# OpenSLAM-org/openslam_g2o

Measured on AMD Instinct MI355X. Metric: linear-solve ms/iter (buildSystem + setLambda + solve + restoreDiagonal), 100k-pose BA, lower is better.
Workload: dtype f64; 1 GPU; synthetic BA (BASELINE.json configs[3]): 100000 poses / 1000000 landmarks / 5000000 observations, BlockSolver_6_3 semantics, Schur + multifrontal block Cholesky, lambda=10; poses=100000, landmarks=1000000, edges=5000000, parallelism=1 GPU, edge_data=estimates+measurements in HBM, errors/Jacobians evaluated inside buildSystem, information=identity, declared for the whole edge set (not read per edge)

## Files before the change

openslam_g2o_amd/csrc/block_solver.h:

```cpp
#pragma once
#include <cstring>
#include <memory>

#include "common.h"
#include "comm.h"
#include "block_pcg.h"
#include "sparse_cholesky.h"

namespace g2ohip {

struct EdgeSet {
  int d = 0, n = 0, dim0 = 0, dim1 = 0;
  bool unary = false;
  int parts = 0;
  std::vector<int> v0, v1;
  int kernel_kind = 0;
  double delta = 1.0;
  DevBuf<double> rk;
  const double *J0 = nullptr, *J1 = nullptr, *omega = nullptr, *err = nullptr;
  DevBuf<double> own_J0, own_J1, own_omega, own_err;
  bool has_data = false;
  bool external = false;
  bool has_err = false;
  DevBuf<int> vp_ptr, vp_ent, vl_ptr, vl_ent;
// ... 283 lines not shown
  void pg_bind_landmark_edges(const char* who, int set, int type, const int* pose_vertex, const int* point_vertex, const double* meas,
                              const double* info, const double* offset, const double* kcam);
  struct EstimateTable {
    DevBuf<double> val, bak;
    DevBuf<int> hidx;
    std::vector<int> h_hidx;
    int n = 0, stride = 0;
    size_t scalars() const { return (size_t)n * stride; }
    bool same(int count, int str, const int* h) const {
      return count == n && str == stride && val.p && std::memcmp(h_hidx.data(), h, sizeof(int) * (size_t)n) == 0;
    }
    void set_values(const double* v, hipStream_t st) { val.upload(v, scalars(), st); }
    void commit(int count, int str, const double* v, const int* h, hipStream_t st) {
      n = count;
      stride = str;
      h_hidx.assign(h, h + count);
      val.upload(v, scalars(), st);
      hidx.upload(h, (size_t)count, st);
      bak.alloc(scalars());
    }
    void push(hipStream_t st) { copy(bak.p, val.p, st); }
    void pop(hipStream_t st) { copy(val.p, bak.p, st); }
    void download(double* h, hipStream_t st) const { val.download(h, scalars(), st); }
    void copy(double* dst, const double* src, hipStream_t st) const {
      if (n > 0) G2OHIP_HIP_CHECK(hipMemcpyAsync(dst, src, scalars() * sizeof(double), hipMemcpyDeviceToDevice, st));
    }
  };
  struct BaFrontEnd {
    int set = -1, n_edges = 0;
    EstimateTable cams, pts;
    double f = 0, cx = 0, cy = 0;
    bool stereo = false;
    double baseline = 0;
    int n_classes = 1;
    DevBuf<double> ctab;
    std::vector<double> h_ctab;
    DevBuf<int> cam_v, pt_v, edge_hpl;
    std::vector<int> h_cam_v, h_pt_v;
    long est_version = 0, bak_version = 0, sys_version = -1;
    int sys_kind = 0;
    double sys_delta = 0.0;
    bool omega_identity = false;
    bool err_valid = false, jac_valid = false;
    DevBuf<double> chi_part;
    bool fused_ok = false;
    DevBuf<double> meas;
    DevBuf<double> meas_pm, omega_pm;
    DevBuf<int> pt_pm, cam_pm;
    DevBuf<double> meas_lm, omega_lm;
    DevBuf<int> cam_q, pt_q;
    DevBuf<double> meas_q, omega_q;
    DevBuf<int> cam_lm, pt_lm, hpl_lm, row_lm;
    DevBuf<int4> ll_rec;
    DevBuf<int> ll_edge;
    DevBuf<int> ll_row;
    DevBuf<double> ll_meas, ll_omega;
    DevBuf<int4> tile_ll;
    DevBuf<int> sel_idx;
    DevBuf<double> sel_out;
    bool ll_slots_ok = false;
    bool has_backup = false;
  } ba_;
  struct PgFrontEnd {
    int set = -1, type = 0;
    DevBuf<int> vi, vj;
    std::vector<int> h_vi, h_vj;
    DevBuf<double> meas;
    EstimateTable poses;
    bool has_backup = false;
    bool err_valid = false, jac_valid = false;
    int lm_set = -1, lm_type = 0;
    DevBuf<int> vp, vl;
    std::vector<int> h_vp, h_vl;
    DevBuf<double> lm_meas;
    EstimateTable points;
    double offset[12] = {1, 0, 0, 0, 1, 0, 0, 0, 1, 0, 0, 0};
    double kcam[4] = {1, 1, 0, 0};
    int pr_set = -1, pr_type = 0;
    DevBuf<int> vq;
    std::vector<int> h_vq;
    DevBuf<double> pr_meas;
    double pr_offset[12] = {1, 0, 0, 0, 1, 0, 0, 0, 1, 0, 0, 0};
  } pg_;
  EventTimer tq_, ts_, tn_, tl_, tb_, tfe_;
  void require_structure() const;
  double reduce_sum_finish(int nblocks);
};

}
```

openslam_g2o_amd/csrc/block_solver.hip:

```cpp
#include "block_solver.h"

#include <algorithm>
#include <atomic>
#include <chrono>
#include <cmath>
#include <cstring>
#include <numeric>

namespace g2ohip {

namespace {

constexpr int kThreads = 256;
constexpr int kMaxBlocks = 1024;

template <int CTRL>
__device__ __forceinline__ double dpp_permute(double v) {
  const int lo = __double2loint(v), hi = __double2hiint(v);
  const int lo2 = __builtin_amdgcn_update_dpp(lo, lo, CTRL, 0xf, 0xf, true);
  const int hi2 = __builtin_amdgcn_update_dpp(hi, hi, CTRL, 0xf, 0xf, true);
  return __hiloint2double(hi2, lo2);
}
template <int G>
__device__ __forceinline__ double group_sum(double v) {
// ... 957 lines not shown
#pragma unroll
  for (int c = 0; c < 3; ++c)
#pragma unroll
    for (int r = 0; r < 3; ++r) {
      double t = 0.0;
#pragma unroll
      for (int m = 0; m < 3; ++m) t += Om[r + 3 * m] * Om[m + 3 * c];
      Om2[r + 3 * c] = t;
    }
  double a, b, cc;
  const bool small = theta < 0.00001;
  if (!small) {
    a = sin(theta) / theta;
    b = (1.0 - cos(theta)) / (theta * theta);
    cc = (theta - sin(theta)) / (theta * theta * theta);
  } else {
    a = 1.0; b = 1.0; cc = 1.0;
  }
#pragma unroll
  for (int i = 0; i < 9; ++i) {
    const double I = (i % 4 == 0) ? 1.0 : 0.0;
    R[i] = I + a * Om[i] + b * Om2[i];
    V[i] = small ? R[i] : I + b * Om[i] + cc * Om2[i];
  }
  double Rn[9], tn[3];
#pragma unroll
  for (int c = 0; c < 3; ++c)
#pragma unroll
    for (int r = 0; r < 3; ++r) {
      double t = 0.0;
#pragma unroll
      for (int m = 0; m < 3; ++m) t += R[r + 3 * m] * T[m + 3 * c];
      Rn[r + 3 * c] = t;
    }
#pragma unroll
  for (int r = 0; r < 3; ++r)
    tn[r] = R[r] * T[9] + R[r + 3] * T[10] + R[r + 6] * T[11] + V[r] * u[3] + V[r + 3] * u[4] + V[r + 6] * u[5];
#pragma unroll
  for (int i = 0; i < 9; ++i) T[i] = Rn[i];
  T[9] = tn[0]; T[10] = tn[1]; T[11] = tn[2];
}
__global__ void __launch_bounds__(kThreads) ba_update_pts_kernel(int np, double* __restrict__ pts, const int* __restrict__ hidx,
                                                               const double* __restrict__ xl) {
  const int t = blockIdx.x * blockDim.x + threadIdx.x;
  if (t >= np * 3) return;
  const int v = t / 3, c = t % 3;
  const int h = hidx[v];
  if (h >= 0) pts[t] += xl[(size_t)h * 3 + c];
}

struct BaEdgeLin {
  double A[6], B[12], r[2], O[4], w;
};
__device__ __forceinline__ void ba_edge_linearize(const double* __restrict__ T, const double* __restrict__ X, const double* __restrict__ z2,
                                                  const double* __restrict__ Op, double f, double cx, double cy, int kind, double delta,
                                                  bool want_A, BaEdgeLin& L) {
  const double x = T[0] * X[0] + T[3] * X[1] + T[6] * X[2] + T[9];
  const double y = T[1] * X[0] + T[4] * X[1] + T[7] * X[2] + T[10];
  const double z = T[2] * X[0] + T[5] * X[1] + T[8] * X[2] + T[11];
  const double iz = 1.0 / z;
  L.r[0] = z2[0] - (x * iz * f + cx);
  L.r[1] = z2[1] - (y * iz * f + cy);
  L.O[0] = Op[0]; L.O[1] = Op[1]; L.O[2] = Op[2]; L.O[3] = Op[3];
  const double Or0 = L.O[0] * L.r[0] + L.O[2] * L.r[1], Or1 = L.O[1] * L.r[0] + L.O[3] * L.r[1];
  L.w = robust_weight(kind, delta, L.r[0] * Or0 + L.r[1] * Or1);
  const double fz = f * iz, xz = x * iz, yz = y * iz;
  if (want_A) {
    const double tmp[6] = {f, 0.0, -xz * f, 0.0, f, -yz * f};
#pragma unroll
    for (int rr = 0; rr < 2; ++rr)
#pragma unroll
      for (int c = 0; c < 3; ++c) {
        double t = 0.0;
#pragma unroll
        for (int m = 0; m < 3; ++m) t += tmp[rr * 3 + m] * T[m + 3 * c];
        L.A[rr + 2 * c] = -iz * t;
      }
  }
  L.B[0 + 2 * 0] = xz * yz * f;          L.B[0 + 2 * 1] = -(1.0 + xz * xz) * f; L.B[0 + 2 * 2] = yz * f;
  L.B[0 + 2 * 3] = -fz;                  L.B[0 + 2 * 4] = 0.0;                  L.B[0 + 2 * 5] = xz * fz;
  L.B[1 + 2 * 0] = (1.0 + yz * yz) * f;  L.B[1 + 2 * 1] = -xz * yz * f;         L.B[1 + 2 * 2] = -xz * f;
  L.B[1 + 2 * 3] = 0.0;                  L.B[1 + 2 * 4] = -fz;                  L.B[1 + 2 * 5] = yz * fz;
}

__device__ __forceinline__ void ba_lm_accumulate(const BaEdgeLin& L, double (&H)[9], double (&b)[3], double (&OA)[6]) {
  const double w = L.w;
  const double O00 = w * L.O[0], O10 = w * L.O[1], O01 = w * L.O[2], O11 = w * L.O[3];
#pragma unroll
  for (int c = 0; c < 3; ++c) {
    OA[0 + 2 * c] = O00 * L.A[0 + 2 * c] + O01 * L.A[1 + 2 * c];
    OA[1 + 2 * c] = O10 * L.A[0 + 2 * c] + O11 * L.A[1 + 2 * c];
  }
  const double Or0 = O00 * L.r[0] + O01 * L.r[1], Or1 = O10 * L.r[0] + O11 * L.r[1];
#pragma unroll
  for (int c = 0; c < 3; ++c) {
    b[c] -= L.A[0 + 2 * c] * Or0 + L.A[1 + 2 * c] * Or1;
#pragma unroll
    for (int a = 0; a < 3; ++a) H[a + 3 * c] += L.A[0 + 2 * a] * OA[0 + 2 * c] + L.A[1 + 2 * a] * OA[1 + 2 * c];
  }
}
__device__ __forceinline__ void ba_hpl_block(const BaEdgeLin& L, const double (&OA)[6], double (&blk)[18]) {
#pragma unroll
  for (int c = 0; c < 3; ++c)
#pragma unroll
    for (int a = 0; a < 6; ++a) blk[a + 6 * c] = L.B[0 + 2 * a] * OA[0 + 2 * c] + L.B[1 + 2 * a] * OA[1 + 2 * c];
}

#ifndef G2OHIP_ASMLM_OCC
#define G2OHIP_ASMLM_OCC 4
#endif
template <int G, bool CLS = false>
__global__ void __launch_bounds__(kThreads, G2OHIP_ASMLM_OCC) ba_assemble_landmarks_kernel(
    int nL, const int* __restrict__ vptr, const int* __restrict__ vent, const double* __restrict__ cams, const double* __restrict__ pts,
    const int* __restrict__ cam_lm, const int* __restrict__ pt_lm, const double* __restrict__ meas_lm, const double* __restrict__ omega_lm,
    const int* __restrict__ hpl_lm, double f, double cx, double cy, int kind, double delta, double* __restrict__ Hll,
    double* __restrict__ bl, double* __restrict__ Hpl, double* __restrict__ err, int ident, const int* __restrict__ pl_colptr,
    int write_hpl, const double* __restrict__ ctab) {
  __shared__ __attribute__((aligned(16))) double stage[kThreads / 64][64 * 18];
// ... 294 lines not shown
    const int* __restrict__ row_lm, double f, double cx, double cy, int kind, double delta, int ident,
    const double* __restrict__ Dinv, const double* __restrict__ bl, const double* __restrict__ xp, double* __restrict__ xl,
    const double* __restrict__ ctab) {
  const int gt = blockIdx.x * blockDim.x + threadIdx.x;
  const int lm = gt / G, g = gt % G;
  const bool active = lm < nL;
  double c[3] = {0.0, 0.0, 0.0};
  const int k0 = active ? vptr[lm] : 0, k1 = active ? vptr[lm + 1] : 0;
  for (int k = k0 + g; k < k1; k += G) {
    const int row = row_lm[k];
    if (row < 0) continue;
    double T[12], X[3], z2[2], Op[4], xv[6];
    const double* Xp = pts + (size_t)pt_lm[k] * 3;
    X[0] = Xp[0]; X[1] = Xp[1]; X[2] = Xp[2];
    load_vec<12>(cams + (size_t)ba_edge_class<CLS>(cam_lm[k], ctab, f, cx, cy, kind, delta) * 12, T);
    load_vec<2>(meas_lm + (size_t)k * 2, z2);
    load_vec<6>(xp + (size_t)row * 6, xv);
    if (ident) {
      Op[0] = Op[3] = 1.0;
      Op[1] = Op[2] = 0.0;
    } else {
      load_vec<4>(omega_lm + (size_t)k * 4, Op);
    }
    BaEdgeLin L;
    ba_edge_linearize(T, X, z2, Op, f, cx, cy, kind, delta, true, L);
    double t0 = 0.0, t1 = 0.0;
#pragma unroll
    for (int a = 0; a < 6; ++a) {
      t0 += L.B[0 + 2 * a] * xv[a];
      t1 += L.B[1 + 2 * a] * xv[a];
    }
    const double w = L.w;
    const double u0 = w * (L.O[0] * t0 + L.O[2] * t1), u1 = w * (L.O[1] * t0 + L.O[3] * t1);
#pragma unroll
    for (int j = 0; j < 3; ++j) c[j] -= L.A[0 + 2 * j] * u0 + L.A[1 + 2 * j] * u1;
  }
  if (G > 1) {
#pragma unroll
    for (int j = 0; j < 3; ++j) c[j] = group_sum<G>(c[j]);
  }
  if (!active || g >= 3) return;
  double cl[3];
#pragma unroll
  for (int j = 0; j < 3; ++j) cl[j] = c[j] + bl[(size_t)lm * 3 + j];
  const double* D = Dinv + (size_t)lm * 9;
  if (G == 1) {
#pragma unroll
    for (int i = 0; i < 3; ++i) xl[(size_t)lm * 3 + i] = D[i] * cl[0] + D[i + 3] * cl[1] + D[i + 6] * cl[2];
  } else {
    xl[(size_t)lm * 3 + g] = D[g] * cl[0] + D[g + 3] * cl[1] + D[g + 6] * cl[2];
  }
}

template <bool CLS>
__global__ void __launch_bounds__(kThreads) ba_back_substitute_slots_kernel(
    const int* __restrict__ tile_lm0, const int4* __restrict__ tile_ll, const int4* __restrict__ ll_rec, const int* __restrict__ ll_row,
    const double* __restrict__ ll_meas, const double* __restrict__ ll_omega, const double* __restrict__ cams,
    const double* __restrict__ pts, double f, double cx, double cy, int kind, double delta, int ident, const double* __restrict__ Dinv,
    const double* __restrict__ bl, const double* __restrict__ xp, double* __restrict__ xl, const double* __restrict__ ctab) {
  const int t = blockIdx.x, tid = threadIdx.x, NT = blockDim.x;
  const int l0 = tile_lm0[(size_t)t * 8];
  const int4 tl = tile_ll[t];
  for (int sb = 0; sb < tl.y; sb += NT) {
    const int si = sb + tid;
    const size_t sg = (size_t)tl.x + min(si, tl.y - 1);
    int4 rc = ll_rec[sg];
    if (si >= tl.y) rc.x = (int)0x80000fffu;
    const int ent = rc.x;
    const int krel = ent & 0xfff, K = (ent >> 12) & 0xff, lmi = (ent >> 20) & 0x7ff;
    const bool head = ent >= 0;
    const int pos = head ? 0 : lmi;
    const int row = krel != 0xfff ? ll_row[sg] : -1;
    double c[3] = {0.0, 0.0, 0.0};
    {
      double T[12], X[3], z2[2], Op[4], xv[6];
      const double* Xp = pts + (size_t)rc.z * 3;
      X[0] = Xp[0]; X[1] = Xp[1]; X[2] = Xp[2];
      load_vec<12>(cams + (size_t)ba_edge_class<CLS>(rc.y, ctab, f, cx, cy, kind, delta) * 12, T);
      load_vec<2>(ll_meas + sg * 2, z2);
      load_vec<6>(xp + (size_t)max(row, 0) * 6, xv);
      if (ident) {
        Op[0] = Op[3] = 1.0;
        Op[1] = Op[2] = 0.0;
      } else {
        load_vec<4>(ll_omega + sg * 4, Op);
      }
      if (row >= 0) {
        BaEdgeLin L;
        ba_edge_linearize(T, X, z2, Op, f, cx, cy, kind, delta, true, L);
        double t0 = 0.0, t1 = 0.0;
#pragma unroll
        for (int a = 0; a < 6; ++a) {
          t0 += L.B[0 + 2 * a] * xv[a];
          t1 += L.B[1 + 2 * a] * xv[a];
        }
        const double w = L.w;
        const double u0 = w * (L.O[0] * t0 + L.O[2] * t1), u1 = w * (L.O[1] * t0 + L.O[3] * t1);
#pragma unroll
        for (int j = 0; j < 3; ++j) c[j] = -(L.A[0 + 2 * j] * u0 + L.A[1 + 2 * j] * u1);
      }
    }
    for (int d = 1; d < tl.w; d <<= 1) {
      const bool take = pos + d < K;
#pragma unroll
      for (int i = 0; i < 3; ++i) {
        const double o = __shfl_down(c[i], d);
        if (take) c[i] += o;
      }
    }
    if (head) {
      const int lm = l0 + lmi;
      double cl[3];
#pragma unroll
      for (int j = 0; j < 3; ++j) cl[j] = c[j] + bl[(size_t)lm * 3 + j];
      const double* D = Dinv + (size_t)lm * 9;
#pragma unroll
      for (int i = 0; i < 3; ++i) xl[(size_t)lm * 3 + i] = D[i] * cl[0] + D[i + 3] * cl[1] + D[i + 6] * cl[2];
    }
  }
}

#ifndef G2OHIP_ASMP_OCC
#define G2OHIP_ASMP_OCC 2
#endif
template <int G, bool CLS = false>
__global__ void __launch_bounds__(kThreads, G2OHIP_ASMP_OCC) ba_assemble_poses_kernel(
    int nP, const int* __restrict__ vptr, const double* __restrict__ cams, const double* __restrict__ pts,
    const int* __restrict__ cam_pm, const int* __restrict__ pt_pm, const double* __restrict__ meas_pm, const double* __restrict__ omega_pm,
    double f, double cx, double cy, int kind, double delta, double* __restrict__ Hpp, const int* __restrict__ diag_blk,
    double* __restrict__ bp, int accumulate, int ident, const int* __restrict__ act, const double* __restrict__ ctab) {
  const int gt = blockIdx.x * blockDim.x + threadIdx.x;
  const int vi_ = gt / G, g = gt % G;
  const bool active = vi_ < nP;
  const int v = (act && active) ? act[vi_] : vi_;
  double H[21], b[6];
#pragma unroll
  for (int i = 0; i < 21; ++i) H[i] = 0.0;
#pragma unroll
  for (int i = 0; i < 6; ++i) b[i] = 0.0;
  const int k0 = active ? vptr[v] : 0, k1 = active ? vptr[v + 1] : 0;
  double T[12];
  const int kf = k0 + g;
  if (kf < k1) load_vec<12>(cams + (size_t)(cam_pm[kf] & (CLS ? 0xffffff : -1)) * 12, T);
  int pt1 = kf < k1 ? pt_pm[kf] : 0, pt2 = kf + G < k1 ? pt_pm[kf + G] : 0;
  double Xn[3] = {0.0, 0.0, 0.0}, z2n[2] = {0.0, 0.0}, Opn[4] = {1.0, 0.0, 0.0, 1.0};
  if (kf < k1) {
    const double* Xp = pts + (size_t)pt1 * 3;
    Xn[0] = Xp[0]; Xn[1] = Xp[1]; Xn[2] = Xp[2];
    load_vec<2>(meas_pm + (size_t)kf * 2, z2n);
    if (!ident) load_vec<4>(omega_pm + (size_t)kf * 4, Opn);
  }
  for (int k = kf; k < k1; k += G) {
    double X[3], z2[2], Op[4];
    X[0] = Xn[0]; X[1] = Xn[1]; X[2] = Xn[2];
    z2[0] = z2n[0]; z2[1] = z2n[1];
#pragma unroll
    for (int i = 0; i < 4; ++i) Op[i] = Opn[i];
    {
      const int kn = k + G, kn2 = k + 2 * G;
      const int pt3 = kn2 < k1 ? pt_pm[kn2] : 0;
      if (kn < k1) {
        const double* Xp = pts + (size_t)pt2 * 3;
        Xn[0] = Xp[0]; Xn[1] = Xp[1]; Xn[2] = Xp[2];
        load_vec<2>(meas_pm + (size_t)kn * 2, z2n);
        if (!ident) load_vec<4>(omega_pm + (size_t)kn * 4, Opn);
      }
      pt2 = pt3;
    }
    if constexpr (CLS) (void)ba_edge_class<true>(cam_pm[k], ctab, f, cx, cy, kind, delta);
    BaEdgeLin L;
    ba_edge_linearize(T, X, z2, Op, f, cx, cy, kind, delta, false, L);
// ... 2293 lines not shown
  return v;
}

double BlockSolver::max_diagonal_sharded() {
  require_structure();
  G2OHIP_HIP_CHECK(hipSetDevice(device_));
  ensure_ll();
  const size_t np = (size_t)nP_ * p_;
  DevBuf<double> diag;
  diag.alloc(np);
  hipLaunchKernelGGL(gather_diag_kernel, dim3(grid_for(np)), dim3(kThreads), 0, st_, nP_, p_, d_Hpp.p, d_pp_diag.p, 0.0, diag.p);
  comm.all_reduce(diag.p, np, 0, st_);
  double m = 0.0;
  {
    const int nblocks = std::min(1024, grid_for(np));
    hipLaunchKernelGGL(max_partial_kernel, dim3(nblocks), dim3(kThreads), 0, st_, np, diag.p, d_red.p);
    std::vector<double> h(nblocks);
    d_red.download(h.data(), nblocks, st_);
    for (double v : h) m = std::max(m, v + lam_pose_);
  }
  double ml = 0.0;
  if (nL_ > 0) {
    const int nblocks = std::min(1024, grid_for((size_t)nL_ * l_));
    hipLaunchKernelGGL(maxdiag_partial_kernel, dim3(nblocks), dim3(kThreads), 0, st_, nL_, l_, d_Hll.p, (const int*)nullptr, d_red.p);
    std::vector<double> h(nblocks);
    d_red.download(h.data(), nblocks, st_);
    for (double v : h) ml = std::max(ml, v + lam_lm_);
  }
  comm.all_reduce_host(&ml, 1, 1, st_);
  return std::max(m, ml);
}

void BlockSolver::partition_info(int* pose_owner, int* block_consumer) {
  require_structure();
  const CholSymbolic& S = chol_->symbolic();
  if (pose_owner) std::copy(S.pose_owner.begin(), S.pose_owner.end(), pose_owner);
  if (block_consumer) std::copy(S.block_consumer.begin(), S.block_consumer.end(), block_consumer);
}

void BlockSolver::solve_back_substitute() {
  require_structure();
  if (!schur_) return;
  G2OHIP_HIP_CHECK(hipSetDevice(device_));
  solve_back_substitute_impl();
}

void BlockSolver::solve_back_substitute_impl() {
  if (profiling) tb_.start(st_);
  const size_t sizeP = (size_t)nP_ * p_;
  prof.begin(KernelProf::kBackSub, st_);
  if (ba_recompute_ok()) {
    EdgeSet& es = *sets_[ba_.set];
    const int GL = ba_lm_group();
    if (ba_fuse_landmarks && ba_.ll_slots_ok && n_tiles_ > 0) {
      with_bool(ba_.n_classes > 1, [&](auto cls) {
        constexpr bool CLS = cls;
        hipLaunchKernelGGL((ba_back_substitute_slots_kernel<CLS>), dim3(n_tiles_), dim3(kThreads), 0, st_, d_tile_lm0.p, ba_.tile_ll.p,
                           ba_.ll_rec.p, ba_.ll_row.p, ba_.ll_meas.p, ba_.ll_omega.p, ba_.cams.val.p, ba_.pts.val.p, ba_.f, ba_.cx, ba_.cy,
                           es.kernel_kind, es.delta, ba_.omega_identity ? 1 : 0, d_Dinv.p, d_b.p + sizeP, d_x.p, d_x.p + sizeP, ba_.ctab.p);
      });
    } else {
      const auto launch = [&](auto g, auto cls) {
        constexpr int GG = g;
        constexpr bool CLS = cls;
        hipLaunchKernelGGL((ba_back_substitute_kernel<GG, CLS>), dim3(grid_for((size_t)nL_ * GG)), dim3(kThreads), 0, st_, nL_, es.vl_ptr.p,
                           ba_.cams.val.p, ba_.pts.val.p, ba_.cam_lm.p, ba_.pt_lm.p, ba_.meas_lm.p, ba_.omega_lm.p, ba_.row_lm.p, ba_.f,
                           ba_.cx, ba_.cy, es.kernel_kind, es.delta, ba_.omega_identity ? 1 : 0, d_Dinv.p, d_b.p + sizeP, d_x.p,
                           d_x.p + sizeP, ba_.ctab.p);
      };
      if (ba_.n_classes > 1) launch(ic<8>, std::true_type{});
      else with_lane_group<1, 4, 8>(GL, [&](auto g) { launch(g, std::false_type{}); });
    }
  } else {
    ensure_hpl();
    const auto row = [&](auto p, auto l) {
      constexpr int P = p, L = l;
      if (p_ != P || l_ != L) return false;
      hipLaunchKernelGGL((back_substitute_kernel<P, L>), dim3(grid_for(nL_)), dim3(kThreads), 0, st_, nL_, d_pl_colptr.p,
                         d_pl_row.p, d_Hpl.p, d_Dinv.p, d_b.p + sizeP, d_x.p, d_x.p + sizeP);
      return true;
    };
    if (!(row(ic<6>, ic<3>) || row(ic<3>, ic<2>) || row(ic<7>, ic<3>) || row(ic<6>, ic<2>) || row(ic<3>, ic<3>)))
      throw ArgFailure("unsupported (pose_dim, landmark_dim)");
  }
  prof.end(KernelProf::kBackSub, st_);
  G2OHIP_HIP_CHECK(hipGetLastError());
  if (profiling) {
    tb_.stop(st_);
    times.backsub = tb_.seconds();
  }
}

template <int PD, int LD>
__global__ void __launch_bounds__(kThreads) mf_pose_kernel(int nP, const int* __restrict__ pm_ptr, const int* __restrict__ pm_q,
                                                         const int* __restrict__ pm_lm, const double* __restrict__ Hpl,
                                                         const double* __restrict__ tl, const double* init,
                                                         const double* __restrict__ dvec, const double* __restrict__ lam, double sign,
                                                         double* out) {
  const int t = blockIdx.x * blockDim.x + threadIdx.x;
  if (t >= nP * PD) return;
  const int i = t / PD, r = t - i * PD;
  double acc = 0.0;
  for (int k = pm_ptr[i]; k < pm_ptr[i + 1]; ++k) {
    const double* B = Hpl + (size_t)pm_q[k] * PD * LD + r;
    const double* tv = tl + (size_t)pm_lm[k] * LD;
#pragma unroll
    for (int c = 0; c < LD; ++c) acc += B[PD * c] * tv[c];
  }
  double v = init[t];
  if (dvec) v += lam[0] * dvec[t];
  out[t] = v + sign * acc;
}
template <int PD, int LD>
// ... 352 lines not shown
      ensure_ll();
      d_Hll.download(h, (size_t)nL_ * l_ * l_, st_);
      if (lam_lm_ != 0.0)
        for (size_t j = 0; j < (size_t)nL_; ++j)
          for (int i = 0; i < l_; ++i) h[j * l_ * l_ + i * (l_ + 1)] += lam_lm_;
      break;
    case 3: ensure_hschur(); d_Hschur.download(h, hs_row.size() * p_ * p_, st_); break;
    case 4: d_Dinv.download(h, (size_t)nL_ * l_ * l_, st_); break;
    default: throw ArgFailure("bad matrix selector");
  }
}
void BlockSolver::ba_set_edges(int set, const int* cam_vertex, const int* point_vertex, const double* meas, const double* info,
                               double f, double cx, double cy) {
  ba_set_edges_classes(set, cam_vertex, point_vertex, meas, info, f, cx, cy, 1, nullptr, nullptr);
}

__global__ void ba_gather_blocks_kernel(size_t n, const int* __restrict__ edge_hpl, const int* __restrict__ cam_v, const int* __restrict__ pt_v,
                                        const double* __restrict__ meas, const double* __restrict__ omega, int* __restrict__ cam_q,
                                        int* __restrict__ pt_q, double* __restrict__ meas_q, double* __restrict__ omega_q) {
  const size_t k = (size_t)blockIdx.x * blockDim.x + threadIdx.x;
  if (k >= n) return;
  const int q = edge_hpl[k];
  if (q < 0) return;
  cam_q[q] = cam_v[k];
  pt_q[q] = pt_v[k];
  meas_q[2 * (size_t)q] = meas[2 * k];
  meas_q[2 * (size_t)q + 1] = meas[2 * k + 1];
  if (omega_q)
    for (int i = 0; i < 4; ++i) omega_q[4 * (size_t)q + i] = omega[4 * k + i];
}
__global__ void ba_gather_lists_kernel(size_t n, const int* __restrict__ ent, const int* __restrict__ cam_v, const int* __restrict__ pt_v,
                                       const double* __restrict__ meas, const double* __restrict__ omega, const int* __restrict__ edge_hpl,
                                       const int* __restrict__ v1, int* __restrict__ cam_o, int* __restrict__ pt_o,
                                       double* __restrict__ meas_o, double* __restrict__ omega_o, int* __restrict__ hpl_o,
                                       int* __restrict__ row_o) {
  const size_t k = (size_t)blockIdx.x * blockDim.x + threadIdx.x;
  if (k >= n) return;
  const size_t e = (size_t)(ent[k] >> 1);
  cam_o[k] = cam_v[e];
  pt_o[k] = pt_v[e];
  meas_o[2 * k] = meas[2 * e];
  meas_o[2 * k + 1] = meas[2 * e + 1];
  if (omega_o)
    for (int i = 0; i < 4; ++i) omega_o[4 * k + i] = omega[4 * e + i];
  if (hpl_o) {
    const int h = edge_hpl[e];
    hpl_o[k] = h;
    row_o[k] = h >= 0 ? v1[e] : -1;
  }
}
__global__ void ba_gather_slots_kernel(const int4* __restrict__ tile_ll, const int* __restrict__ slots, const int* __restrict__ vl_ent,
                                       const int* __restrict__ cam_lm, const int* __restrict__ pt_lm, const int* __restrict__ hpl_lm,
                                       const int* __restrict__ row_lm, const double* __restrict__ meas_lm, const double* __restrict__ omega_lm,
                                       int4* __restrict__ rec, int* __restrict__ edge, int* __restrict__ srow, double* __restrict__ ms,
                                       double* __restrict__ os) {
  const int4 tl = tile_ll[blockIdx.x];
  for (int i = threadIdx.x; i < tl.y; i += blockDim.x) {
    const size_t sidx = (size_t)tl.x + i;
    const int w = slots[sidx];
    int4 r = make_int4(w, 0, 0, -1);
    int ed = 0, row = -1;
    double m0 = 0.0, m1 = 0.0, o[4] = {0.0, 0.0, 0.0, 0.0};
    if ((w & 0xfff) != 0xfff) {
      const size_t k = (size_t)tl.z + (w & 0xfff);
      r = make_int4(w, cam_lm[k], pt_lm[k], hpl_lm[k]);
      ed = vl_ent[k] >> 1;
      row = row_lm[k];
      m0 = meas_lm[2 * k];
      m1 = meas_lm[2 * k + 1];
      if (os)
        for (int j = 0; j < 4; ++j) o[j] = omega_lm[4 * k + j];
    }
    rec[sidx] = r;
    edge[sidx] = ed;
    srow[sidx] = row;
    ms[2 * sidx] = m0;
    ms[2 * sidx + 1] = m1;
    if (os)
      for (int j = 0; j < 4; ++j) os[4 * sidx + j] = o[j];
  }
}

void BlockSolver::ba_set_edges_classes(int set, const int* cam_vertex, const int* point_vertex, const double* meas, const double* info,
                                       double f, double cx, double cy, int n_classes, const double* class_params, const int* edge_class) {
  invalidate_graphs();
  require_structure();
  if (set < 0 || set >= (int)sets_.size()) throw ArgFailure("bad edge set id");
  EdgeSet& es = *sets_[set];
  if (es.d != 2 || es.unary || es.dim0 != 3 || es.dim1 != 6 || p_ != 6 || l_ != 3)
    throw ArgFailure("ba_set_edges: the set must be EdgeProjectXYZ2UV-shaped (d=2, vertex0 = 3-dof point, vertex1 = 6-dof pose)");
  if (!cam_vertex || !point_vertex || !meas) throw ArgFailure("ba_set_edges: null array");
  G2OHIP_HIP_CHECK(hipSetDevice(device_));
  const size_t n = (size_t)es.n;
  const bool lapt = getenv("G2OHIP_SETUP_TIMING") != nullptr;
  auto lap_now = [] { return std::chrono::duration<double>(std::chrono::steady_clock::now().time_since_epoch()).count(); };
  double lap_t = lap_now();
  auto lap = [&](const char* what) {
    if (!lapt) return;
    const double t = lap_now();
    fprintf(stderr, "ba_set_edges: %-37s %.3f s\n", what, t - lap_t);
    lap_t = t;
  };
  if (n_classes < 1 || n_classes > 128) throw ArgFailure("ba_set_edges_classes: 1 to 128 edge classes");
  if (n_classes > 1 && (!class_params || !edge_class)) throw ArgFailure("ba_set_edges_classes: null class table");
  if (es.rk.p)
    throw StateFailure("ba_set_edges: the set carries per-edge robust kernels (set_robust_kernel_per_edge); on the BA front end they go through ba_set_edges_classes -- clear them first");
  std::vector<int> camc;
  if (n_classes > 1) {
    for (int c = 0; c < n_classes; ++c) {
      const double kd = class_params[5 * c + 3];
      if (!(kd == 0.0 || kd == 1.0 || kd == 2.0 || kd == 3.0 || kd == 4.0 || kd == 5.0)) throw ArgFailure("ba_set_edges_classes: robust kernel kind of a class must be 0..5");
      if (kd != 0.0 && !(class_params[5 * c + 4] > 0.0)) throw ArgFailure("ba_set_edges_classes: robust kernel delta of class " + std::to_string(c) + " must be positive");
    }
    camc.resize(n);
    for (size_t k = 0; k < n; ++k) {
      if (edge_class[k] < 0 || edge_class[k] >= n_classes) throw ArgFailure("ba_set_edges_classes: class of edge " + std::to_string(k) + " outside the table");
      if (cam_vertex[k] < 0 || cam_vertex[k] >= (1 << 24)) throw ArgFailure("ba_set_edges_classes: camera indices are limited to 2^24 with edge classes");
      camc[k] = cam_vertex[k] | (edge_class[k] << 24);
    }
  }
  ba_validate_edges(es, cam_vertex, point_vertex, n, ba_.cams.h_hidx.data(), ba_.cams.n, ba_.pts.h_hidx.data(), ba_.pts.n);
  std::vector<int> edge_hpl(n, -1);
  bool unique = es.first_lm && es.first_ol;
  {
    std::vector<char> seen(pl_row.size(), 0);
    for (size_t k = 0; k < n; ++k)
// ... 105 lines not shown
        for (int lm = l0; lm < l1; ++lm) {
          const int K = es.h_vl_ptr[lm + 1] - es.h_vl_ptr[lm], lmi = lm - l0;
          if (K > 64 || lmi >= 0x7ff || es.h_vl_ptr[lm + 1] - kb >= 0xfff) return -1;
          const int need = std::max(K, 1);
          if (used + need > 64) {
            if (out)
              for (int i = used; i < 64; ++i) out[total + i - used] = kIdleSlot;
            total += 64 - used;
            used = 0;
          }
          if (out) {
            if (K == 0) out[total] = 0xfff | (lmi << 20);
            for (int j = 0; j < K; ++j)
              out[total + j] = (es.h_vl_ptr[lm] + j - kb) | (K << 12) | (j == 0 ? (lmi << 20) : (int)(0x80000000u | ((unsigned)j << 20)));
          }
          total += need;
          used = (used + need) & 63;
          kmax = std::max(kmax, K);
        }
        if (used) {
          if (out)
            for (int i = used; i < 64; ++i) out[total + i - used] = kIdleSlot;
          total += 64 - used;
        }
        return total;
      };
      host_parallel_for((size_t)n_tiles_, [&](size_t t0_, size_t t1_) {
        for (size_t t = t0_; t < t1_; ++t) {
          int kmax = 0;
          const int c = walk((int)t, nullptr, kmax);
          if (c < 0) okf.store(false);
          cnt[t] = std::max(c, 0);
        }
      }, 64);
      size_t ns = 0;
      for (int t = 0; t < n_tiles_; ++t) {
        tl[t].x = (int)ns;
        ns += (size_t)cnt[t];
      }
      if (okf.load() && ns < ((size_t)1 << 31)) {
        std::vector<int> slots(std::max<size_t>(ns, 1), kIdleSlot);
        host_parallel_for((size_t)n_tiles_, [&](size_t t0_, size_t t1_) {
          for (size_t t = t0_; t < t1_; ++t) {
            int kmax = 0;
            walk((int)t, slots.data() + tl[t].x, kmax);
            tl[t] = make_int4(tl[t].x, cnt[t], es.h_vl_ptr[tile_lm0_h_[t]], kmax);
          }
        }, 64);
        const size_t nsa = slots.size();
        DevBuf<int> d_slots;
        d_slots.upload(slots, st_);
        ba_.tile_ll.upload(tl, st_);
        ba_.ll_rec.alloc(nsa);
        ba_.ll_edge.alloc(nsa);
        ba_.ll_row.alloc(nsa);
        ba_.ll_meas.alloc(nsa * 2);
        if (d_omega) ba_.ll_omega.alloc(nsa * 4);
        if (ns == 0) {
          const int4 idle = make_int4(kIdleSlot, 0, 0, -1);
          const int none = -1;
          ba_.ll_rec.upload(&idle, 1, st_);
          ba_.ll_row.upload(&none, 1, st_);
          ba_.ll_edge.zero(st_);
          ba_.ll_meas.zero(st_);
        } else {
          hipLaunchKernelGGL(ba_gather_slots_kernel, dim3(n_tiles_), dim3(kThreads), 0, st_, ba_.tile_ll.p, d_slots.p, es.vl_ent.p, ba_.cam_lm.p,
                             ba_.pt_lm.p, ba_.hpl_lm.p, ba_.row_lm.p, ba_.meas_lm.p, d_omega ? ba_.omega_lm.p : (const double*)nullptr,
                             ba_.ll_rec.p, ba_.ll_edge.p, ba_.ll_row.p, ba_.ll_meas.p, d_omega ? ba_.ll_omega.p : (double*)nullptr);
        }
        G2OHIP_HIP_CHECK(hipGetLastError());
        G2OHIP_HIP_CHECK(hipStreamSynchronize(st_));
        ba_.ll_slots_ok = true;
      }
    }
    lap("lane slots of the tiles");
    G2OHIP_HIP_CHECK(hipStreamSynchronize(st_));
  }
  lap("pose-major / landmark-major uploads");
  if (!(ba_fused && ba_.fused_ok)) {
    es.own_J0.alloc(n * 6);
    es.own_J1.alloc(n * 12);
  }
  es.own_err.alloc(n * 2);
  es.J0 = es.own_J0.p; es.J1 = es.own_J1.p; es.omega = es.own_omega.p; es.err = es.own_err.p;
  es.has_data = false;
  prepare_ba_tile_kernels();
  G2OHIP_HIP_CHECK(hipStreamSynchronize(st_));
  lap("buffers, kernel attributes, sync");
}

void BlockSolver::ba_set_stereo_edges(int set, const int* cam_vertex, const int* point_vertex, const double* meas, const double* info,
                                      double f, double cx, double cy, double baseline) {
  invalidate_graphs();
  require_structure();
  if (set < 0 || set >= (int)sets_.size()) throw ArgFailure("bad edge set id");
  EdgeSet& es = *sets_[set];
  if (es.d != 3 || es.unary || es.dim0 != 3 || es.dim1 != 6 || p_ != 6 || l_ != 3)
    throw ArgFailure("ba_set_stereo_edges: the set must be EdgeProjectXYZ2UVU-shaped (d=3, vertex0 = 3-dof point, vertex1 = 6-dof pose)");
  if (!cam_vertex || !point_vertex || !meas) throw ArgFailure("ba_set_stereo_edges: null array");
  if (!std::isfinite(f) || !std::isfinite(cx) || !std::isfinite(cy) || !std::isfinite(baseline))
    throw ArgFailure("ba_set_stereo_edges: non-finite camera parameters");
  if (f == 0.0) throw ArgFailure("ba_set_stereo_edges: the focal length must not be zero");
  if (es.rk.p)
    throw StateFailure("ba_set_stereo_edges: the set carries per-edge robust kernels (set_robust_kernel_per_edge) -- clear them first and set them again on the bound set");
  G2OHIP_HIP_CHECK(hipSetDevice(device_));
  const size_t n = (size_t)es.n;
  ba_validate_edges(es, cam_vertex, point_vertex, n, ba_.cams.h_hidx.data(), ba_.cams.n, ba_.pts.h_hidx.data(), ba_.pts.n);
  ba_.set = set;
  ba_.n_edges = es.n;
  ba_.f = f; ba_.cx = cx; ba_.cy = cy;
  ba_.stereo = true;
  ba_.baseline = baseline;
  ba_.n_classes = 1;
  ba_.h_ctab.clear();
  ba_.ctab.release();
  ba_.h_cam_v.assign(cam_vertex, cam_vertex + n);
  ba_.h_pt_v.assign(point_vertex, point_vertex + n);
  ba_.err_valid = ba_.jac_valid = false;
  chi2_valid_ = false;
  ba_.sys_version = -1;
  ba_.fused_ok = false;
  ba_.ll_slots_ok = false;
  for (DevBuf<int>* b : {&ba_.edge_hpl, &ba_.pt_pm, &ba_.cam_pm, &ba_.cam_q, &ba_.pt_q, &ba_.cam_lm, &ba_.pt_lm, &ba_.hpl_lm, &ba_.row_lm,
                         &ba_.ll_edge, &ba_.ll_row})
    b->release();
  for (DevBuf<double>* b : {&ba_.meas_pm, &ba_.omega_pm, &ba_.meas_lm, &ba_.omega_lm, &ba_.meas_q, &ba_.omega_q, &ba_.ll_meas, &ba_.ll_omega})
    b->release();
  ba_.ll_rec.release();
  ba_.tile_ll.release();
  ba_.cam_v.upload(cam_vertex, n, st_);
  ba_.pt_v.upload(point_vertex, n, st_);
  ba_.meas.upload(meas, n * 3, st_);
  ba_.omega_identity = info == nullptr;
  if (!info) {
    es.own_omega.alloc(n * 9);
    if (n) hipLaunchKernelGGL(identity3_kernel, dim3(grid_for(n * 9)), dim3(kThreads), 0, st_, n, es.own_omega.p);
  } else {
    es.own_omega.upload(info, n * 9, st_);
  }
  es.own_J0.alloc(n * 9);
  es.own_J1.alloc(n * 18);
  es.own_err.alloc(n * 3);
  es.J0 = es.own_J0.p; es.J1 = es.own_J1.p; es.omega = es.own_omega.p; es.err = es.own_err.p;
  es.external = false;
  es.has_data = false;
  es.has_err = false;
  G2OHIP_HIP_CHECK(hipGetLastError());
  G2OHIP_HIP_CHECK(hipStreamSynchronize(st_));
}

bool BlockSolver::ba_recompute_ok() const {
  if (!schur_ || p_ != 6 || l_ != 3 || ba_.set < 0 || !ba_fused || !ba_.fused_ok || ba_.cams.n <= 0) return false;
  if (ba_.sys_version < 0 || ba_.sys_version != ba_.est_version) return false;
  const EdgeSet& bs = *sets_[ba_.set];
  if (bs.kernel_kind != ba_.sys_kind || bs.delta != ba_.sys_delta) return false;
  for (size_t i = 0; i < sets_.size(); ++i)
    if ((int)i != ba_.set && sets_[i]->n > 0 && sets_[i]->touches_lm) return false;
  return true;
}

void BlockSolver::ba_validate_edges(const EdgeSet& es, const int* cam_v, const int* pt_v, size_t n, const int* cam_hidx, int nc,
                                    const int* pt_hidx, int np) const {
  if (n == 0 || nc == 0) return;
  for (size_t k = 0; k < n; ++k) {
    const int c = cam_v[k], q = pt_v[k];
    if (c < 0 || c >= nc) throw ArgFailure("ba: camera index " + std::to_string(c) + " of edge " + std::to_string(k) + " outside the estimate table");
    if (q < 0 || q >= np) throw ArgFailure("ba: point index " + std::to_string(q) + " of edge " + std::to_string(k) + " outside the estimate table");
    const int hc = cam_hidx[c], hp = pt_hidx[q];
    if (hc >= nP_ || hp >= nL_) throw ArgFailure("ba: hessian index of an estimate outside the structure");
    const int v1 = hc < 0 ? -1 : hc, v0 = hp < 0 ? -1 : nP_ + hp;
    if (es.v1[k] != v1 || es.v0[k] != v0)
      throw ArgFailure("ba: edge " + std::to_string(k) + " connects vertices (" + std::to_string(es.v0[k]) + ", " + std::to_string(es.v1[k]) +
                       ") in the edge set but estimates with hessian indices (" + std::to_string(v0) + ", " + std::to_string(v1) + ")");
  }
}

void BlockSolver::pg_validate(const EdgeSet& es, const int* vi, const int* vj, size_t n, const int* hidx, int nv) const {
  if (n == 0 || nv == 0) return;
  for (size_t k = 0; k < n; ++k) {
    const int a = vi[k], b = vj[k];
    if (a < 0 || a >= nv || b < 0 || b >= nv) throw ArgFailure("pg: vertex index of edge " + std::to_string(k) + " outside the estimate table");
// ... 619 lines not shown
```

Baseline: 1.133 ms/iter.

## Slim back-substitution slot records and prefetch next slot metadata

The fused landmark back-substitution kernel now reads a compact int2 record in place of the int4 slot record. It takes the camera row from the camera hidx array, loads the point position once per landmark head and broadcasts it across lanes with shuffles, and prefetches the next records two iterations ahead. For non-robust kernels it skips the residual and robust-weight computation and the measurement load, and the reduction loop now stops on a wave-wide any() test. This cuts memory traffic and latency in back-substitution, at the cost of an extra host pass at setup to verify that each landmark has a single point, plus extra buffers.

```diff
diff --git a/openslam_g2o_amd/csrc/block_solver.h b/openslam_g2o_amd/csrc/block_solver.h
--- a/openslam_g2o_amd/csrc/block_solver.h
+++ b/openslam_g2o_amd/csrc/block_solver.h
@@ -359,6 +359,9 @@
     DevBuf<double> meas_q, omega_q;
     DevBuf<int> cam_lm, pt_lm, hpl_lm, row_lm;
     DevBuf<int4> ll_rec;
+    DevBuf<int2> ll_rec2;
+    DevBuf<int> lm_pt;
+    bool ll_one_point = false;
     DevBuf<int> ll_edge;
     DevBuf<int> ll_row;
     DevBuf<double> ll_meas, ll_omega;
diff --git a/openslam_g2o_amd/csrc/block_solver.hip b/openslam_g2o_amd/csrc/block_solver.hip
--- a/openslam_g2o_amd/csrc/block_solver.hip
+++ b/openslam_g2o_amd/csrc/block_solver.hip
@@ -1033,6 +1033,7 @@
 struct BaEdgeLin {
   double A[6], B[12], r[2], O[4], w;
 };
+template <bool WANT_R = true>
 __device__ __forceinline__ void ba_edge_linearize(const double* __restrict__ T, const double* __restrict__ X, const double* __restrict__ z2,
                                                   const double* __restrict__ Op, double f, double cx, double cy, int kind, double delta,
                                                   bool want_A, BaEdgeLin& L) {
@@ -1040,11 +1041,15 @@
   const double y = T[1] * X[0] + T[4] * X[1] + T[7] * X[2] + T[10];
   const double z = T[2] * X[0] + T[5] * X[1] + T[8] * X[2] + T[11];
   const double iz = 1.0 / z;
-  L.r[0] = z2[0] - (x * iz * f + cx);
-  L.r[1] = z2[1] - (y * iz * f + cy);
   L.O[0] = Op[0]; L.O[1] = Op[1]; L.O[2] = Op[2]; L.O[3] = Op[3];
-  const double Or0 = L.O[0] * L.r[0] + L.O[2] * L.r[1], Or1 = L.O[1] * L.r[0] + L.O[3] * L.r[1];
-  L.w = robust_weight(kind, delta, L.r[0] * Or0 + L.r[1] * Or1);
+  if constexpr (WANT_R) {
+    L.r[0] = z2[0] - (x * iz * f + cx);
+    L.r[1] = z2[1] - (y * iz * f + cy);
+    const double Or0 = L.O[0] * L.r[0] + L.O[2] * L.r[1], Or1 = L.O[1] * L.r[0] + L.O[3] * L.r[1];
+    L.w = robust_weight(kind, delta, L.r[0] * Or0 + L.r[1] * Or1);
+  } else {
+    L.w = 1.0;
+  }
   const double fz = f * iz, xz = x * iz, yz = y * iz;
   if (want_A) {
     const double tmp[6] = {f, 0.0, -xz * f, 0.0, f, -yz * f};
@@ -1445,32 +1450,44 @@
   }
 }
 
-template <bool CLS>
+template <bool CLS, bool ROBUST>
 __global__ void __launch_bounds__(kThreads) ba_back_substitute_slots_kernel(
-    const int* __restrict__ tile_lm0, const int4* __restrict__ tile_ll, const int4* __restrict__ ll_rec, const int* __restrict__ ll_row,
-    const double* __restrict__ ll_meas, const double* __restrict__ ll_omega, const double* __restrict__ cams,
+    const int* __restrict__ tile_lm0, const int4* __restrict__ tile_ll, const int2* __restrict__ ll_rec2, const int* __restrict__ cam_row,
+    const int* __restrict__ lm_pt, const double* __restrict__ ll_meas, const double* __restrict__ ll_omega, const double* __restrict__ cams,
     const double* __restrict__ pts, double f, double cx, double cy, int kind, double delta, int ident, const double* __restrict__ Dinv,
     const double* __restrict__ bl, const double* __restrict__ xp, double* __restrict__ xl, const double* __restrict__ ctab) {
   const int t = blockIdx.x, tid = threadIdx.x, NT = blockDim.x;
   const int l0 = tile_lm0[(size_t)t * 8];
   const int4 tl = tile_ll[t];
+  if (tl.y <= 0) return;
+  const auto rec_at = [&](int sb_) {
+    const int si = sb_ + tid;
+    int2 r = ll_rec2[(size_t)tl.x + min(si, tl.y - 1)];
+    if (si >= tl.y) r.x = (int)0x80000fffu;
+    return r;
+  };
+  const auto row_of = [&](const int2& r) { return (r.x & 0xfff) != 0xfff ? cam_row[CLS ? (r.y & 0xffffff) : r.y] : -1; };
+  const auto pt_of = [&](const int2& r) { return r.x >= 0 ? lm_pt[l0 + ((r.x >> 20) & 0x7ff)] : 0; };
+  int2 rc = rec_at(0), rc_n = rec_at(NT);
+  int row = row_of(rc), pt = pt_of(rc);
   for (int sb = 0; sb < tl.y; sb += NT) {
-    const int si = sb + tid;
-    const size_t sg = (size_t)tl.x + min(si, tl.y - 1);
-    int4 rc = ll_rec[sg];
-    if (si >= tl.y) rc.x = (int)0x80000fffu;
+    const size_t sg = (size_t)tl.x + min(sb + tid, tl.y - 1);
     const int ent = rc.x;
-    const int krel = ent & 0xfff, K = (ent >> 12) & 0xff, lmi = (ent >> 20) & 0x7ff;
+    const int K = (ent >> 12) & 0xff, lmi = (ent >> 20) & 0x7ff;
     const bool head = ent >= 0;
     const int pos = head ? 0 : lmi;
-    const int row = krel != 0xfff ? ll_row[sg] : -1;
+    const int ci = ba_edge_class<CLS>(rc.y, ctab, f, cx, cy, kind, delta);
     double c[3] = {0.0, 0.0, 0.0};
+    int2 rc_nn;
+    int row_n, pt_n;
     {
-      double T[12], X[3], z2[2], Op[4], xv[6];
-      const double* Xp = pts + (size_t)rc.z * 3;
-      X[0] = Xp[0]; X[1] = Xp[1]; X[2] = Xp[2];
-      load_vec<12>(cams + (size_t)ba_edge_class<CLS>(rc.y, ctab, f, cx, cy, kind, delta) * 12, T);
-      load_vec<2>(ll_meas + sg * 2, z2);
+      double T[12], X[3] = {0.0, 0.0, 0.0}, z2[2] = {0.0, 0.0}, Op[4], xv[6];
+      if (head) {
+        const double* Xp = pts + (size_t)pt * 3;
+        X[0] = Xp[0]; X[1] = Xp[1]; X[2] = Xp[2];
+      }
+      load_vec<12>(cams + (size_t)ci * 12, T);
+      if constexpr (ROBUST) load_vec<2>(ll_meas + sg * 2, z2);
       load_vec<6>(xp + (size_t)max(row, 0) * 6, xv);
       if (ident) {
         Op[0] = Op[3] = 1.0;
@@ -1478,9 +1495,16 @@
       } else {
         load_vec<4>(ll_omega + sg * 4, Op);
       }
+      rc_nn = rec_at(sb + 2 * NT);
+      row_n = row_of(rc_n);
+      pt_n = pt_of(rc_n);
+      {
+        const int src = (tid & 63) - pos;
+        X[0] = __shfl(X[0], src); X[1] = __shfl(X[1], src); X[2] = __shfl(X[2], src);
+      }
       if (row >= 0) {
         BaEdgeLin L;
-        ba_edge_linearize(T, X, z2, Op, f, cx, cy, kind, delta, true, L);
+        ba_edge_linearize<ROBUST>(T, X, z2, Op, f, cx, cy, kind, delta, true, L);
         double t0 = 0.0, t1 = 0.0;
 #pragma unroll
         for (int a = 0; a < 6; ++a) {
@@ -1493,7 +1517,7 @@
         for (int j = 0; j < 3; ++j) c[j] = -(L.A[0 + 2 * j] * u0 + L.A[1 + 2 * j] * u1);
       }
     }
-    for (int d = 1; d < tl.w; d <<= 1) {
+    for (int d = 1; __any(pos + d < K); d <<= 1) {
       const bool take = pos + d < K;
 #pragma unroll
       for (int i = 0; i < 3; ++i) {
@@ -1510,6 +1534,8 @@
 #pragma unroll
       for (int i = 0; i < 3; ++i) xl[(size_t)lm * 3 + i] = D[i] * cl[0] + D[i + 3] * cl[1] + D[i + 6] * cl[2];
     }
+    rc = rc_n; rc_n = rc_nn;
+    row = row_n; pt = pt_n;
   }
 }
 
@@ -3909,13 +3935,16 @@
   if (ba_recompute_ok()) {
     EdgeSet& es = *sets_[ba_.set];
     const int GL = ba_lm_group();
-    if (ba_fuse_landmarks && ba_.ll_slots_ok && n_tiles_ > 0) {
-      with_bool(ba_.n_classes > 1, [&](auto cls) {
-        constexpr bool CLS = cls;
-        hipLaunchKernelGGL((ba_back_substitute_slots_kernel<CLS>), dim3(n_tiles_), dim3(kThreads), 0, st_, d_tile_lm0.p, ba_.tile_ll.p,
-                           ba_.ll_rec.p, ba_.ll_row.p, ba_.ll_meas.p, ba_.ll_omega.p, ba_.cams.val.p, ba_.pts.val.p, ba_.f, ba_.cx, ba_.cy,
-                           es.kernel_kind, es.delta, ba_.omega_identity ? 1 : 0, d_Dinv.p, d_b.p + sizeP, d_x.p, d_x.p + sizeP, ba_.ctab.p);
-      });
+    if (ba_fuse_landmarks && ba_.ll_slots_ok && ba_.ll_one_point && n_tiles_ > 0) {
+      const auto launch = [&](auto cls, auto robust) {
+        constexpr bool CLS = cls, ROBUST = robust;
+        hipLaunchKernelGGL((ba_back_substitute_slots_kernel<CLS, ROBUST>), dim3(n_tiles_), dim3(kThreads), 0, st_, d_tile_lm0.p, ba_.tile_ll.p,
+                           ba_.ll_rec2.p, ba_.cams.hidx.p, ba_.lm_pt.p, ba_.ll_meas.p, ba_.ll_omega.p, ba_.cams.val.p, ba_.pts.val.p, ba_.f,
+                           ba_.cx, ba_.cy, es.kernel_kind, es.delta, ba_.omega_identity ? 1 : 0, d_Dinv.p, d_b.p + sizeP, d_x.p,
+                           d_x.p + sizeP, ba_.ctab.p);
+      };
+      if (ba_.n_classes > 1) launch(std::true_type{}, std::true_type{});
+      else with_bool(es.kernel_kind != 0, [&](auto robust) { launch(std::false_type{}, robust); });
     } else {
       const auto launch = [&](auto g, auto cls) {
         constexpr int GG = g;
@@ -4374,8 +4403,8 @@
 __global__ void ba_gather_slots_kernel(const int4* __restrict__ tile_ll, const int* __restrict__ slots, const int* __restrict__ vl_ent,
                                        const int* __restrict__ cam_lm, const int* __restrict__ pt_lm, const int* __restrict__ hpl_lm,
                                        const int* __restrict__ row_lm, const double* __restrict__ meas_lm, const double* __restrict__ omega_lm,
-                                       int4* __restrict__ rec, int* __restrict__ edge, int* __restrict__ srow, double* __restrict__ ms,
-                                       double* __restrict__ os) {
+                                       int4* __restrict__ rec, int2* __restrict__ rec2, int* __restrict__ edge, int* __restrict__ srow,
+                                       double* __restrict__ ms, double* __restrict__ os) {
   const int4 tl = tile_ll[blockIdx.x];
   for (int i = threadIdx.x; i < tl.y; i += blockDim.x) {
     const size_t sidx = (size_t)tl.x + i;
@@ -4394,6 +4423,7 @@
         for (int j = 0; j < 4; ++j) o[j] = omega_lm[4 * k + j];
     }
     rec[sidx] = r;
+    rec2[sidx] = make_int2(r.x, r.y);
     edge[sidx] = ed;
     srow[sidx] = row;
     ms[2 * sidx] = m0;
@@ -4605,6 +4635,7 @@
         d_slots.upload(slots, st_);
         ba_.tile_ll.upload(tl, st_);
         ba_.ll_rec.alloc(nsa);
+        ba_.ll_rec2.alloc(nsa);
         ba_.ll_edge.alloc(nsa);
         ba_.ll_row.alloc(nsa);
         ba_.ll_meas.alloc(nsa * 2);
@@ -4612,14 +4643,32 @@
         if (ns == 0) {
           const int4 idle = make_int4(kIdleSlot, 0, 0, -1);
           const int none = -1;
+          const int2 idle2 = make_int2(kIdleSlot, 0);
           ba_.ll_rec.upload(&idle, 1, st_);
+          ba_.ll_rec2.upload(&idle2, 1, st_);
           ba_.ll_row.upload(&none, 1, st_);
           ba_.ll_edge.zero(st_);
           ba_.ll_meas.zero(st_);
         } else {
           hipLaunchKernelGGL(ba_gather_slots_kernel, dim3(n_tiles_), dim3(kThreads), 0, st_, ba_.tile_ll.p, d_slots.p, es.vl_ent.p, ba_.cam_lm.p,
                              ba_.pt_lm.p, ba_.hpl_lm.p, ba_.row_lm.p, ba_.meas_lm.p, d_omega ? ba_.omega_lm.p : (const double*)nullptr,
-                             ba_.ll_rec.p, ba_.ll_edge.p, ba_.ll_row.p, ba_.ll_meas.p, d_omega ? ba_.ll_omega.p : (double*)nullptr);
+                             ba_.ll_rec.p, ba_.ll_rec2.p, ba_.ll_edge.p, ba_.ll_row.p, ba_.ll_meas.p, d_omega ? ba_.ll_omega.p : (double*)nullptr);
+        }
+        {
+          std::vector<int> lm_pt((size_t)std::max(nL_, 1), 0);
+          std::atomic<bool> one_point(true);
+          host_parallel_for((size_t)nL_, [&](size_t b_, size_t e_) {
+            for (size_t lm = b_; lm < e_; ++lm) {
+              const int k0 = es.h_vl_ptr[lm], k1 = es.h_vl_ptr[lm + 1];
+              if (k0 == k1) continue;
+              const int pt = ba_.h_pt_v[(size_t)(es.h_vl_ent[k0] >> 1)];
+              for (int k = k0 + 1; k < k1; ++k)
+                if (ba_.h_pt_v[(size_t)(es.h_vl_ent[k] >> 1)] != pt) one_point.store(false);
+              lm_pt[lm] = pt;
+            }
+          });
+          ba_.lm_pt.upload(lm_pt, st_);
+          ba_.ll_one_point = one_point.load();
         }
         G2OHIP_HIP_CHECK(hipGetLastError());
         G2OHIP_HIP_CHECK(hipStreamSynchronize(st_));
@@ -4680,6 +4729,8 @@
   for (DevBuf<double>* b : {&ba_.meas_pm, &ba_.omega_pm, &ba_.meas_lm, &ba_.omega_lm, &ba_.meas_q, &ba_.omega_q, &ba_.ll_meas, &ba_.ll_omega})
     b->release();
   ba_.ll_rec.release();
+  ba_.ll_rec2.release();
+  ba_.lm_pt.release();
   ba_.tile_ll.release();
   ba_.cam_v.upload(cam_vertex, n, st_);
   ba_.pt_v.upload(point_vertex, n, st_);
```

After: 1.124 ms/iter, median of 6. About the same (-0.8%).
